# bauerca/maxwell

Measured on NVIDIA B200. Metric: curlcurl_spmv_crs_equiv_gbs, higher is better.
Workload: dtype f64

## Files before the change

### maxwell_b200/csrc/mxg_internal.h

```cpp
#pragma once
#include <cuda_runtime.h>
#include <nccl.h>

#include <cstdarg>
#include <cstdint>
#include <cstdio>
#include <memory>
#include <string>
#include <vector>

#include "mxgpu.h"

namespace mxg {

void setError(const char* fmt, ...);

#define MXG_CUDA(expr)                                                                       \
  do {                                                                                       \
    cudaError_t e_ = (expr);                                                                 \
    if (e_ != cudaSuccess) {                                                                 \
      mxg::setError("%s:%d: %s failed: %s", __FILE__, __LINE__, #expr, cudaGetErrorString(e_)); \
      return MXG_ERR_CUDA;                                                                   \
    }                                                                                        \
  } while (0)
// ... 94 lines not shown
  size_t bytes = 0;
  ~MvStorage();
};

struct mxg_mv {
  mxg_map* map = nullptr;
  bool isComplex = false;
  int ncols = 0;
  int64_t ld = 0;
  std::shared_ptr<MvStorage> storage;
  std::vector<void*> col;
  std::vector<int> baseCol;
};

namespace mxg {
struct HaloPeer {
  int rank = -1;
  int64_t sendCount = 0, sendOffset = 0;
  int64_t recvCount = 0, recvStart = 0;
};
}

struct mxg_crs {
  mxg_ctx* ctx = nullptr;
  mxg_map *rowMap = nullptr, *domMap = nullptr;
  bool isComplex = false;
  int64_t nRows = 0, nLoc = 0, nnz = 0;
  int64_t gLo = 0, gHi = 0;
  int32_t* dRowPat = nullptr;
  int32_t* dPatOff = nullptr;
  void* dPat = nullptr;
  int64_t numPats = 0, dictRows = 0, patEntries = 0;
  int64_t nGen = 0, ellEntries = 0;
  int32_t* dGenRow = nullptr;
  int32_t* dGenLen = nullptr;
  int64_t* dSlicePtr = nullptr;
  int32_t* dCol = nullptr;
  void* dVal = nullptr;
  int64_t intBegin = 0, intEnd = 0, genIntBegin = 0, genIntEnd = 0;
  int64_t ghostRows = 0;
  std::vector<mxg::HaloPeer> peers;
  int32_t* dSendIdx = nullptr;
  int64_t sendTotal = 0;
  mutable void* dSendBuf = nullptr;
  mutable void* dGhost = nullptr;
  mutable int haloCols = 0;
  size_t deviceBytes = 0;
  void* dInvDiag = nullptr;
  int ilv = 1;
  void* dWinTiles = nullptr;
  int winR = 0;
  int winIlv = 1;
  int winMaxVec = 1;
  int64_t winTiles = 0, winValid = 0;
  int64_t winBufElems = 0;
  struct GraphEntry {
    uint64_t key;
    cudaGraphExec_t exec;
    int launches;
  };
  mutable std::vector<GraphEntry> graphs;
  struct P2P {
    bool on = false;
    unsigned long long hostEpoch = 0;
    int capCols = 0;
    void* ghost = nullptr;
    unsigned long long* flags = nullptr;
    unsigned int* done = nullptr;
    void* dArgs = nullptr;
    unsigned long long* trace = nullptr;
    int npeers = 0;
    int peerRank[8];
    void* peerGhost[8];
    unsigned long long* peerFlag[8];
    int64_t remoteStart[8], remoteGTot[8];
    std::vector<void*> opened;
  };
  mutable P2P p2p;
};

namespace mxg {
template <class T>
inline ColTable<T> tableOf(const mxg_mv* mv, int first = 0, int count = -1) {
  ColTable<T> t;
  if (count < 0) count = mv->ncols - first;
  for (int j = 0; j < count; ++j) t.p[j] = static_cast<T*>(mv->col[first + j]);
  return t;
}
int ensureScratch(mxg_ctx* ctx, size_t bytes);
int ensurePinned(mxg_ctx* ctx, size_t bytes);
int allReduceScratch(mxg_ctx* ctx, size_t count);
int mapGlobalCount(mxg_map* map, int64_t* out);
int checkHaloFault(const mxg_ctx* ctx, const char* where);
int crsCreateFromDevice(mxg_map* rowMap, mxg_map* domMap, const int64_t* dRowptr, const int32_t* dCol, const void* dVal, int64_t colBegin,
                        int64_t colFieldSize, const int64_t* colFieldGids, int isComplex, int layout, mxg_crs** out);
inline int gridFor(const mxg_ctx* ctx, int64_t work, int block, int perSM) {
  int64_t need = (work + block - 1) / block;
  int64_t cap = int64_t(ctx->numSMs) * perSM;
  if (need < 1) need = 1;
  return int(need < cap ? need : cap);
}
}
```

### maxwell_b200/csrc/mxg_spmm_win.cuh

```cuda
#pragma once
#include <algorithm>
#include <climits>
#include <cstdint>
#include <vector>

namespace mxg {

constexpr int kWinThreads = 384;

struct alignas(16) WinTile {
  int32_t segLo[3];
  int32_t segLen[3];
  int32_t shift[3];
  int32_t dLo, dHi;
  int32_t valid;
  int32_t total;
  int32_t pad[3];
};
static_assert(sizeof(WinTile) == 64, "WinTile layout");

template <class Delta>
inline std::vector<WinTile> planWinTiles(const int32_t* rowPat, const int32_t* patOff, int64_t numPats, Delta delta, int64_t nRows,
                                         int64_t nLoc, int R, int align, int64_t budgetElems, int64_t* maxTotal, int64_t* validTiles) {
  const int64_t nTiles = (nRows + R - 1) / R;
// ... 42 lines not shown
    if (!a) { a = b; b = 0; }
    const size_t n = ents.size();
    size_t cb[4];
    int ncl;
    if (a && b) { cb[0] = 0; cb[1] = a; cb[2] = b; cb[3] = n; ncl = 3; }
    else if (a) { cb[0] = 0; cb[1] = a; cb[2] = n; ncl = 2; }
    else { cb[0] = 0; cb[1] = n; ncl = 1; }
    int cls[3];
    if (ncl == 3) { cls[0] = 0; cls[1] = 1; cls[2] = 2; W.dLo = int32_t(ents[a].d); W.dHi = int32_t(ents[b - 1].d); }
    else if (ncl == 2) { cls[0] = 1; cls[1] = 2; W.dHi = int32_t(ents[a - 1].d); }
    else cls[0] = 1;
    bool ok = true;
    int64_t lo[3], hi[3];
    for (int c = 0; c < ncl; ++c) {
      lo[c] = INT64_MAX;
      hi[c] = INT64_MIN;
      for (size_t i = cb[c]; i < cb[c + 1]; ++i) { lo[c] = std::min(lo[c], ents[i].lo); hi[c] = std::max(hi[c], ents[i].hi); }
      if (lo[c] < 0 || hi[c] > nLoc) ok = false;
      lo[c] = lo[c] / align * align;
      hi[c] = (hi[c] + align - 1) / align * align;
    }
    int order[3] = {0, 1, 2};
    std::sort(order, order + ncl, [&](int x, int y) { return lo[x] < lo[y]; });
    int64_t total = 0;
    int nseg = 0, segOf[3] = {0, 0, 0};
    int64_t segLo[3] = {0, 0, 0}, segHi[3] = {0, 0, 0}, segOff[3] = {0, 0, 0};
    for (int k = 0; k < ncl && ok; ++k) {
      const int c = order[k];
      if (nseg > 0 && lo[c] <= segHi[nseg - 1]) segHi[nseg - 1] = std::max(segHi[nseg - 1], hi[c]);
      else { segLo[nseg] = lo[c]; segHi[nseg] = hi[c]; ++nseg; }
      segOf[c] = nseg - 1;
    }
    for (int sgi = 0; sgi < nseg && ok; ++sgi) {
      segOff[sgi] = total;
      total += segHi[sgi] - segLo[sgi];
      W.segLo[sgi] = int32_t(segLo[sgi]);
      W.segLen[sgi] = int32_t(segHi[sgi] - segLo[sgi]);
    }
    for (int c = 0; c < ncl && ok; ++c) W.shift[cls[c]] = int32_t(segOff[segOf[c]] - segLo[segOf[c]]);
    if (!ok || total > budgetElems || total >= (int64_t(1) << 30)) {
      W = WinTile{};
      W.dLo = INT_MIN;
      W.dHi = INT_MAX;
      continue;
    }
    W.valid = 1;
    W.total = int32_t(total);
    *maxTotal = std::max<int64_t>(*maxTotal, total);
    ++*validTiles;
  }
  return tiles;
}

#ifdef __CUDACC__
__device__ __forceinline__ uint32_t smemU32(const void* p) { return static_cast<uint32_t>(__cvta_generic_to_shared(p)); }
__device__ __forceinline__ void mbarInit(uint64_t* bar, uint32_t count) {
  asm volatile("mbarrier.init.shared::cta.b64 [%0], %1;" ::"r"(smemU32(bar)), "r"(count) : "memory");
}
__device__ __forceinline__ void mbarFenceInit() {
  asm volatile("fence.mbarrier_init.release.cluster;" ::: "memory");
  asm volatile("fence.proxy.async.shared::cta;" ::: "memory");
}
__device__ __forceinline__ void mbarExpectTx(uint64_t* bar, uint32_t bytes) {
  asm volatile("mbarrier.arrive.expect_tx.shared::cta.b64 _, [%0], %1;" ::"r"(smemU32(bar)), "r"(bytes) : "memory");
}
__device__ __forceinline__ void bulkLoad(void* dstSmem, const void* srcGlobal, uint32_t bytes, uint64_t* bar) {
  asm volatile("cp.async.bulk.shared::cluster.global.mbarrier::complete_tx::bytes [%0], [%1], %2, [%3];" ::"r"(smemU32(dstSmem)),
               "l"(srcGlobal), "r"(bytes), "r"(smemU32(bar))
               : "memory");
}
__device__ __forceinline__ void mbarWait(uint64_t* bar, uint32_t parity) {
  uint32_t done;
  do {
    asm volatile(
        "{\n"
        ".reg .pred p;\n"
        "mbarrier.try_wait.parity.shared::cta.b64 p, [%1], %2;\n"
        "selp.u32 %0, 1, 0, p;\n"
        "}\n"
        : "=r"(done)
        : "r"(smemU32(bar)), "r"(parity)
        : "memory");
  } while (!done);
}
#endif

}
```

### maxwell_b200/csrc/mxg_spmv.cu

```cuda
#include <algorithm>
#include <cstdlib>
#include <cstring>

#include "mxg_internal.h"
#include "mxg_ilv_model.h"
#include "mxg_order.h"
#include "mxg_spmm_win.cuh"
#include "mxg_scan.cuh"

using namespace mxg;

namespace {

constexpr int kBlock = 256;

template <class T>
struct PatEntry;
template <>
struct __align__(16) PatEntry<double> {
  double v;
  int32_t d;
  int32_t pad;
};
template <>
// ... 118 lines not shown
        v[u] = S.val[at];
      }
#pragma unroll
      for (int u = 0; u < kUnroll; ++u)
#pragma unroll
        for (int jj = 0; jj < NV; ++jj)
          xv[u][jj] = loadX<T, GHOST>(X, min(j0 + jj, nvec - 1), c[u]);
#pragma unroll
      for (int u = 0; u < kUnroll; ++u)
        if (k + u < len) {
#pragma unroll
          for (int jj = 0; jj < NV; ++jj) accum(acc[jj], v[u], xv[u][jj]);
        }
    }
    if (row >= 0) {
#pragma unroll
      for (int jj = 0; jj < NV; ++jj)
        if (NV == 1 || j0 + jj < nvec) storeY(Y.p[j0 + jj], row, acc[jj], ep);
    }
  }
}

template <class T, bool GHOST>
__device__ __forceinline__ void sellRowSimple(int64_t i, const SellArgs<T>& S, const XSource<T>& X, const ColTable<T>& Y, int nvec,
                                              const Epilogue<T>& ep) {
  const int64_t row = S.genRow[i];
  if (row < 0) return;
  const int len = S.genLen[i];
  const int64_t base = S.slicePtr[i >> 5] + (i & 31);
  for (int j = 0; j < nvec; ++j) {
    T acc = zeroOf<T>();
    for (int k = 0; k < len; ++k) accum(acc, S.val[base + int64_t(k) * 32], loadX<T, GHOST>(X, j, S.col[base + int64_t(k) * 32]));
    storeY(Y.p[j], row, acc, ep);
  }
}

template <class T, bool GHOST, int NV>
__global__ void __launch_bounds__(kBlock) k_spmm_dict(int64_t rowBegin, int64_t rowEnd, DictArgs<T> D,
                                                      XSource<T> X, ColTable<T> Y, int nvec, Epilogue<T> ep) {
  const int64_t row = rowBegin + blockIdx.x * int64_t(kBlock) + threadIdx.x;
  if (row < rowEnd) dictRow<T, GHOST, NV>(row, D, X, Y, nvec, ep);
}

constexpr int kBlockIlv = 384;
template <class T, bool GHOST, int NV>
__global__ void __launch_bounds__(kBlockIlv) k_spmm_dict_ilv3(int64_t rowBegin, int64_t rowEnd, DictArgs<T> D,
                                                              XSource<T> X, ColTable<T> Y, int nvec, Epilogue<T> ep) {
  const int warp = threadIdx.x >> 5, lane = threadIdx.x & 31;
  const int64_t row = rowBegin + blockIdx.x * int64_t(kBlockIlv) + (warp / 3) * 96 + 3 * lane + (warp % 3);
  if (row < rowEnd) dictRow<T, GHOST, NV>(row, D, X, Y, nvec, ep);
}


template <class T>
__device__ __forceinline__ void winIssue(const WinTile& W, const T* __restrict__ xcol, T* buf, uint64_t* bar) {
  uint32_t bytes = 0;
#pragma unroll
  for (int sgi = 0; sgi < 3; ++sgi) bytes += uint32_t(W.segLen[sgi]) * uint32_t(sizeof(T));
  mbarExpectTx(bar, bytes);
  int off = 0;
#pragma unroll
  for (int sgi = 0; sgi < 3; ++sgi) {
    if (W.segLen[sgi] > 0) bulkLoad(buf + off, xcol + W.segLo[sgi], uint32_t(W.segLen[sgi]) * uint32_t(sizeof(T)), bar);
    off += W.segLen[sgi];
  }
}

constexpr int kWinSlot = 16;

template <class T>
__device__ __forceinline__ PatEntry<T> ldEntry(const PatEntry<T>* p) {
  PatEntry<T> e;
  const int4* s = reinterpret_cast<const int4*>(p);
  int4* d = reinterpret_cast<int4*>(&e);
#pragma unroll
  for (int i = 0; i < int(sizeof(PatEntry<T>) / 16); ++i) d[i] = s[i];
  return e;
}

struct WinShift {
  int32_t dLo, dHi, s0, s1, s2;
};
template <class T>
__device__ __forceinline__ T winRowDot(const PatEntry<T>* __restrict__ ent, int32_t len, int32_t r, const T* __restrict__ xs, const WinShift& w) {
  T acc = zeroOf<T>();
  int32_t q = 0;
  for (; q + 1 < len; q += 2) {
    const PatEntry<T> e0 = ldEntry<T>(ent + q);
    const PatEntry<T> e1 = ldEntry<T>(ent + q + 1);
    const T x0 = xs[r + e0.d + (e0.d < w.dLo ? w.s0 : (e0.d > w.dHi ? w.s2 : w.s1))];
    const T x1 = xs[r + e1.d + (e1.d < w.dLo ? w.s0 : (e1.d > w.dHi ? w.s2 : w.s1))];
    accum(acc, entryVal(e0), x0);
    accum(acc, entryVal(e1), x1);
  }
  if (q < len) {
    const PatEntry<T> e0 = ldEntry<T>(ent + q);
    accum(acc, entryVal(e0), xs[r + e0.d + (e0.d < w.dLo ? w.s0 : (e0.d > w.dHi ? w.s2 : w.s1))]);
  }
  return acc;
}

template <class T, int ILV, int RPT>
__global__ void __launch_bounds__(kWinThreads) k_spmm_win(int64_t rowBegin, int64_t rowEnd, int64_t tile0, DictArgs<T> D,
                                                          const WinTile* __restrict__ tiles, XSource<T> X, ColTable<T> Y, int nvec,
                                                          Epilogue<T> ep) {
  extern __shared__ __align__(128) unsigned char smemRaw[];
  uint64_t* bar = reinterpret_cast<uint64_t*>(smemRaw);
  WinTile* Ws = reinterpret_cast<WinTile*>(smemRaw + 64);
  PatEntry<T>* slots = reinterpret_cast<PatEntry<T>*>(smemRaw + 128);
  constexpr int kWarps = kWinThreads / 32;
  T* buf = reinterpret_cast<T*>(smemRaw + 128 + sizeof(PatEntry<T>) * kWarps * RPT * kWinSlot);
  constexpr int R = kWinThreads * RPT;
  const int64_t tile = tile0 + blockIdx.x;
  if (threadIdx.x == 0) {
    const int4* src = reinterpret_cast<const int4*>(tiles + tile);
    int4* dst = reinterpret_cast<int4*>(Ws);
#pragma unroll
    for (int i = 0; i < 4; ++i) dst[i] = __ldg(src + i);
    mbarInit(bar, 1);
    mbarFenceInit();
    if (Ws->valid) winIssue<T>(*Ws, X.x.p[0], buf, bar);
  }
  const int warp = threadIdx.x >> 5, lane = threadIdx.x & 31;
  const int tOff = ILV == 3 ? (warp / 3) * 96 + 3 * lane + (warp % 3) : int(threadIdx.x);
  int64_t row[RPT];
  int32_t o[RPT], len[RPT];
  bool uni[RPT];
#pragma unroll
  for (int i = 0; i < RPT; ++i) {
    row[i] = tile * R + i * kWinThreads + tOff;
    int32_t p = -1;
    if (row[i] >= rowBegin && row[i] < rowEnd) p = D.rowPat[row[i]];
    o[i] = len[i] = 0;
    if (p >= 0) { o[i] = __ldg(D.patOff + p); len[i] = __ldg(D.patOff + p + 1) - o[i]; }
    const int32_t pmax = __reduce_max_sync(0xffffffffu, p);
    uni[i] = __all_sync(0xffffffffu, p < 0 || p == pmax) && pmax >= 0;
    const int32_t oU = __shfl_sync(0xffffffffu, o[i], __ffs(__ballot_sync(0xffffffffu, p == pmax)) - 1);
    const int32_t lenU = __shfl_sync(0xffffffffu, len[i], __ffs(__ballot_sync(0xffffffffu, p == pmax)) - 1);
    uni[i] = uni[i] && lenU <= kWinSlot;
    if (uni[i] && lane < lenU) slots[(warp * RPT + i) * kWinSlot + lane] = ldEntry<T>(D.pat + oU + lane);
  }
  __syncthreads();
  if (!Ws->valid) {
#pragma unroll
    for (int i = 0; i < RPT; ++i)
      if (row[i] >= rowBegin && row[i] < rowEnd) dictRow<T, false, 1>(row[i], D, X, Y, nvec, ep);
    return;
  }
  const int32_t dLo = Ws->dLo, dHi = Ws->dHi, s0 = Ws->shift[0], s1 = Ws->shift[1], s2 = Ws->shift[2];
  for (int j = 0; j < nvec; ++j) {
    mbarWait(bar, j & 1);
    const T* __restrict__ xs = buf;
#pragma unroll
    for (int i = 0; i < RPT; ++i) {
      if (len[i] == 0) continue;
      const int32_t r = int32_t(row[i]);
      const WinShift ws{dLo, dHi, s0, s1, s2};
      const T acc = uni[i] ? winRowDot<T>(slots + (warp * RPT + i) * kWinSlot, len[i], r, xs, ws)
                           : winRowDot<T>(D.pat + o[i], len[i], r, xs, ws);
      storeY(Y.p[j], row[i], acc, ep);
    }
    if (j + 1 < nvec) {
      __syncthreads();
      if (threadIdx.x == 0) winIssue<T>(*Ws, X.x.p[j + 1], buf, bar);
    }
  }
}

template <class T, bool GHOST, int NV>
__global__ void __launch_bounds__(kBlock) k_spmm_sell(int64_t genBegin, int64_t genEnd, SellArgs<T> S,
                                                      XSource<T> X, ColTable<T> Y, int nvec, Epilogue<T> ep) {
  const int64_t i = genBegin + blockIdx.x * int64_t(kBlock) + threadIdx.x;
  if (i < genEnd) sellRow<T, GHOST, NV>(i, S, X, Y, nvec, ep);
}

struct Segments {
  int64_t begin[4], end[4];
  int blockStart[5];
};
template <class T, bool GHOST, int NV>
__global__ void __launch_bounds__(kBlock) k_spmm_multi(Segments G, DictArgs<T> D, SellArgs<T> S,
                                                       XSource<T> X, ColTable<T> Y, int nvec, Epilogue<T> ep) {
  int seg = 0;
  while (seg < 3 && int(blockIdx.x) >= G.blockStart[seg + 1]) ++seg;
  const int64_t idx = G.begin[seg] + int64_t(int(blockIdx.x) - G.blockStart[seg]) * kBlock + threadIdx.x;
  if (idx >= G.end[seg]) return;
  if (seg < 2) dictRow<T, GHOST, NV>(idx, D, X, Y, nvec, ep);
  else sellRow<T, GHOST, NV>(idx, S, X, Y, nvec, ep);
}

template <class T>
__global__ void __launch_bounds__(kBlock) k_pack(ColTable<T> x, const int32_t* __restrict__ idx, int64_t n, T* __restrict__ buf) {
  const T* __restrict__ c = x.p[blockIdx.y];
  for (int64_t i = blockIdx.x * int64_t(kBlock) + threadIdx.x; i < n; i += int64_t(gridDim.x) * kBlock)
    buf[blockIdx.y * n + i] = c[idx[i]];
}

#define LAUNCH_CHECK(ctx)         \
  do {                            \
    (ctx)->launches++;            \
    MXG_CUDA(cudaGetLastError()); \
  } while (0)

template <class T>
DictArgs<T> dictArgs(const mxg_crs* A) { return {A->dRowPat, A->dPatOff, static_cast<const PatEntry<T>*>(A->dPat)}; }
template <class T>
SellArgs<T> sellArgs(const mxg_crs* A) { return {A->dGenRow, A->dGenLen, A->dSlicePtr, A->dCol, static_cast<const T*>(A->dVal)}; }

template <class T, bool GHOST>
int launchSegments(const mxg_crs* A, const int64_t b[4], const int64_t e[4], const XSource<T>& X, const ColTable<T>& Y, int nvec,
                   const Epilogue<T>& ep, cudaStream_t st) {
  mxg_ctx* ctx = A->ctx;
  Segments G;
  int blocks = 0;
  for (int sgm = 0; sgm < 4; ++sgm) {
    G.begin[sgm] = b[sgm];
    G.end[sgm] = e[sgm] > b[sgm] ? e[sgm] : b[sgm];
    G.blockStart[sgm] = blocks;
    blocks += int((G.end[sgm] - G.begin[sgm] + kBlock - 1) / kBlock);
  }
  G.blockStart[4] = blocks;
  if (blocks == 0) return MXG_OK;
  const DictArgs<T> D = dictArgs<T>(A);
  const SellArgs<T> S = sellArgs<T>(A);
  if (nvec == 1) k_spmm_multi<T, GHOST, 1><<<blocks, kBlock, 0, st>>>(G, D, S, X, Y, nvec, ep);
  else if (nvec == 2) k_spmm_multi<T, GHOST, 2><<<blocks, kBlock, 0, st>>>(G, D, S, X, Y, nvec, ep);
  else k_spmm_multi<T, GHOST, 4><<<blocks, kBlock, 0, st>>>(G, D, S, X, Y, nvec, ep);
  LAUNCH_CHECK(ctx);
  return MXG_OK;
}


template <class T> struct WinCfg;
template <> struct WinCfg<double> { static constexpr int RPT = 2; };
template <> struct WinCfg<zd> { static constexpr int RPT = 1; };
constexpr size_t kWinSmemMax = 200 * 1024;
constexpr size_t kWinBufBudget = 100 * 1024;
template <class T>
constexpr size_t winSmemHeader() { return 128 + sizeof(PatEntry<T>) * (kWinThreads / 32) * WinCfg<T>::RPT * kWinSlot; }

template <class T>
int launchWin(const mxg_crs* A, int64_t rowBegin, int64_t rowEnd, const XSource<T>& X, const ColTable<T>& Y, int nvec,
              const Epilogue<T>& ep, cudaStream_t st) {
  mxg_ctx* ctx = A->ctx;
  constexpr int RPT = WinCfg<T>::RPT;
  const int R = A->winR;
  const int64_t tile0 = rowBegin / R, tiles = (rowEnd + R - 1) / R - tile0;
  const size_t smem = winSmemHeader<T>() + size_t(A->winBufElems) * sizeof(T);
  const DictArgs<T> D = dictArgs<T>(A);
  const WinTile* wt = static_cast<const WinTile*>(A->dWinTiles);
  static bool attrSet[2] = {false, false};
  if (A->winIlv == 3) {
    auto kern = k_spmm_win<T, 3, RPT>;
    if (!attrSet[0]) { MXG_CUDA(cudaFuncSetAttribute(kern, cudaFuncAttributeMaxDynamicSharedMemorySize, int(kWinSmemMax))); attrSet[0] = true; }
    kern<<<unsigned(tiles), kWinThreads, smem, st>>>(rowBegin, rowEnd, tile0, D, wt, X, Y, nvec, ep);
  } else {
    auto kern = k_spmm_win<T, 1, RPT>;
    if (!attrSet[1]) { MXG_CUDA(cudaFuncSetAttribute(kern, cudaFuncAttributeMaxDynamicSharedMemorySize, int(kWinSmemMax))); attrSet[1] = true; }
    kern<<<unsigned(tiles), kWinThreads, smem, st>>>(rowBegin, rowEnd, tile0, D, wt, X, Y, nvec, ep);
  }
  LAUNCH_CHECK(ctx);
  return MXG_OK;
}

template <class T, bool GHOST>
int launchRange(const mxg_crs* A, int64_t rowBegin, int64_t rowEnd, int64_t genBegin, int64_t genEnd, const XSource<T>& X,
                const ColTable<T>& Y, int nvec, const Epilogue<T>& ep, bool marks) {
  mxg_ctx* ctx = A->ctx;
  const cudaStream_t st = ctx->stream;
  if (marks) MXG_CUDA(cudaEventRecord(ctx->prof[1], st));
  if (A->dictRows > 0 && rowEnd > rowBegin && A->winR > 0 && nvec <= A->winMaxVec) {
    const int rc = launchWin<T>(A, rowBegin, rowEnd, X, Y, nvec, ep, st);
    if (rc) return rc;
  } else if (A->dictRows > 0 && rowEnd > rowBegin) {
    const DictArgs<T> D = dictArgs<T>(A);
    if (A->ilv == 3) {
      const int64_t blocks = (rowEnd - rowBegin + kBlockIlv - 1) / kBlockIlv;
      if (nvec == 1) k_spmm_dict_ilv3<T, GHOST, 1><<<blocks, kBlockIlv, 0, st>>>(rowBegin, rowEnd, D, X, Y, nvec, ep);
      else if (nvec == 2) k_spmm_dict_ilv3<T, GHOST, 2><<<blocks, kBlockIlv, 0, st>>>(rowBegin, rowEnd, D, X, Y, nvec, ep);
      else k_spmm_dict_ilv3<T, GHOST, 4><<<blocks, kBlockIlv, 0, st>>>(rowBegin, rowEnd, D, X, Y, nvec, ep);
    } else {
      const int64_t blocks = (rowEnd - rowBegin + kBlock - 1) / kBlock;
      if (nvec == 1) k_spmm_dict<T, GHOST, 1><<<blocks, kBlock, 0, st>>>(rowBegin, rowEnd, D, X, Y, nvec, ep);
      else if (nvec == 2) k_spmm_dict<T, GHOST, 2><<<blocks, kBlock, 0, st>>>(rowBegin, rowEnd, D, X, Y, nvec, ep);
      else k_spmm_dict<T, GHOST, 4><<<blocks, kBlock, 0, st>>>(rowBegin, rowEnd, D, X, Y, nvec, ep);
    }
    LAUNCH_CHECK(ctx);
  }
  if (marks) MXG_CUDA(cudaEventRecord(ctx->prof[2], st));
  if (genEnd > genBegin) {
    const int64_t blocks = (genEnd - genBegin + kBlock - 1) / kBlock;
    const SellArgs<T> S = sellArgs<T>(A);
    if (nvec == 1) k_spmm_sell<T, GHOST, 1><<<blocks, kBlock, 0, st>>>(genBegin, genEnd, S, X, Y, nvec, ep);
    else if (nvec == 2) k_spmm_sell<T, GHOST, 2><<<blocks, kBlock, 0, st>>>(genBegin, genEnd, S, X, Y, nvec, ep);
    else k_spmm_sell<T, GHOST, 4><<<blocks, kBlock, 0, st>>>(genBegin, genEnd, S, X, Y, nvec, ep);
    LAUNCH_CHECK(ctx);
  }
  if (marks) MXG_CUDA(cudaEventRecord(ctx->prof[3], st));
  return MXG_OK;
}

template <class T>
int launchBoundary(const mxg_crs* A, const XSource<T>& X, const ColTable<T>& Y, int nvec, const Epilogue<T>& ep, cudaStream_t st) {
  const int64_t b[4] = {0, A->intEnd, 0, A->genIntEnd};
  const int64_t e[4] = {A->dictRows > 0 ? A->intBegin : 0, A->dictRows > 0 ? A->nRows : A->intEnd, A->genIntBegin, A->nGen};
  return launchSegments<T, true>(A, b, e, X, Y, nvec, ep, st);
}

__host__ __device__ inline uint64_t mix64(uint64_t h, uint64_t v) {
  h ^= v + 0x9E3779B97F4A7C15ull + (h << 6) + (h >> 2);
  h *= 0xBF58476D1CE4E5B9ull;
  return h ^ (h >> 29);
}
// ... 416 lines not shown
    for (int64_t i = 0; i < cnt[q]; ++i) {
      const int64_t g = all[size_t(q) * maxCnt + i];
      if (g >= domLo && g <= domHi) {
        const int32_t l = domLookup[g];
        MXG_REQUIRE(l >= 0, "mxg_crs_create: rank %d asks for GID %lld which lies in rank %d's range but is not in its map",
                    q, (long long)g, ctx->rank);
        sendIdx.push_back(l);
      }
    }
    peer.sendCount = int64_t(sendIdx.size()) - peer.sendOffset;
    const int64_t qLo = ranges[2 * q], qHi = ranges[2 * q + 1];
    if (qLo <= qHi) {
      auto b = std::lower_bound(ghosts.begin(), ghosts.end(), qLo);
      auto e = std::upper_bound(ghosts.begin(), ghosts.end(), qHi);
      peer.recvStart = int64_t(b - ghosts.begin());
      peer.recvCount = int64_t(e - b);
    }
    if (peer.sendCount > 0 || peer.recvCount > 0) A->peers.push_back(peer);
  }
  int64_t covered = 0;
  for (const Peer& p : A->peers) covered += p.recvCount;
  MXG_REQUIRE(covered == int64_t(ghosts.size()), "mxg_crs_create: %lld ghost columns have no owner",
              (long long)(int64_t(ghosts.size()) - covered));
  A->sendTotal = int64_t(sendIdx.size());
  int rcU = uploadVec(sendIdx, &A->dSendIdx, &A->deviceBytes, ctx);
  if (rcU) return rcU;
  return setupP2P(A, int64_t(ghosts.size()));
}

template <class T>
int planKernels(mxg_crs* A, const std::vector<int32_t>& rowPat, const std::vector<int32_t>& patOff, const std::vector<PatEntry<T>>& pat) {
  mxg_ctx* ctx = A->ctx;
  const int64_t nRows = A->nRows, nLoc = A->nLoc;
  int rc = MXG_OK;
  {
    const char* env = std::getenv("MXG_SPMV_ILV");
    const std::string mode = env ? env : "auto";
    A->ilv = 1;
    if (mode == "3") A->ilv = 3;
    else if (mode != "1" && A->dictRows > 0) {
      const PatEntry<T>* pe = pat.data();
      const mxg::IlvCost cost = mxg::ilvCostModel(rowPat.data(), patOff.data(), [pe](int32_t q) { return pe[q].d; }, A->intBegin,
                                                  A->intEnd, int(sizeof(T)), int(sizeof(PatEntry<T>)));
      if (mxg::ilvWins(cost)) A->ilv = 3;
    }
  }

  {
    const char* env = std::getenv("MXG_SPMV_WIN");
    const bool want = !(env && std::strcmp(env, "0") == 0);
    if (want && A->dictRows > 0 && nLoc + A->gLo + A->gHi < (int64_t(1) << 30)) {
      constexpr int R = kWinThreads * WinCfg<T>::RPT;
      constexpr int align = 16 / int(sizeof(T)) > 0 ? 16 / int(sizeof(T)) : 1;
      const PatEntry<T>* pe = pat.data();
      int64_t maxTotal = 0, valid = 0;
      std::vector<WinTile> tiles = planWinTiles(rowPat.data(), patOff.data(), A->numPats, [pe](int32_t q) { return int64_t(pe[q].d); }, nRows,
                                                nLoc, R, align, int64_t(std::min(kWinBufBudget, kWinSmemMax - winSmemHeader<T>()) / sizeof(T)), &maxTotal, &valid);
      if (valid > 0) {
        WinTile* dT = nullptr;
        if ((rc = uploadVec(tiles, &dT, &A->deviceBytes, ctx))) return rc;
        A->dWinTiles = dT;
        A->winR = R;
        A->winTiles = int64_t(tiles.size());
        A->winValid = valid;
        A->winBufElems = maxTotal;
        A->winMaxVec = 1;
        if (const char* mv = std::getenv("MXG_WIN_MAXVEC")) A->winMaxVec = std::atoi(mv);
        int64_t same1 = 0, same3 = 0;
        for (int64_t r = 0; r + 3 < nRows; ++r) {
          if (rowPat[r] < 0) continue;
          same1 += rowPat[r] == rowPat[r + 1];
          same3 += rowPat[r] == rowPat[r + 3];
        }
        A->winIlv = same3 > same1 ? 3 : 1;
        if (const char* iv = std::getenv("MXG_SPMV_ILV")) {
          if (std::strcmp(iv, "1") == 0) A->winIlv = 1;
          if (std::strcmp(iv, "3") == 0) A->winIlv = 3;
        }
      }
    }
  }

  return rc;
}

struct Scratch {
  std::vector<void*> p;
  ~Scratch() { for (void* q : p) if (q) cudaFree(q); }
  template <class U>
  U* get(int64_t n) {
    void* q = nullptr;
    if (cudaMalloc(&q, size_t(n > 0 ? n : 1) * sizeof(U)) != cudaSuccess) { cudaGetLastError(); return nullptr; }
    p.push_back(q);
    return static_cast<U*>(q);
  }
};

constexpr unsigned long long kLbEmpty = 0xFFFFFFFFFFFFFFFFull;

__global__ void k_lb_mark_ghosts(const int32_t* __restrict__ col, int64_t cnt, int64_t c0, int64_t c1, int32_t* __restrict__ flag) {
  for (int64_t q = int64_t(blockIdx.x) * blockDim.x + threadIdx.x; q < cnt; q += int64_t(gridDim.x) * blockDim.x) {
    const int64_t l = col[q];
    if (l < c0 || l >= c1) flag[l] = 1;
  }
}
__global__ void k_lb_compact(const int32_t* __restrict__ flag, const int64_t* __restrict__ off, int64_t n, int32_t* __restrict__ list) {
  for (int64_t i = int64_t(blockIdx.x) * blockDim.x + threadIdx.x; i < n; i += int64_t(gridDim.x) * blockDim.x)
    if (flag[i]) list[off[i]] = int32_t(i);
}
__global__ void k_lb_ext(const int64_t* __restrict__ rp, const int32_t* __restrict__ colG, int64_t nRows, int64_t base, int64_t c0,
                         int64_t c1, int64_t nLoc, int64_t gLo, const int64_t* __restrict__ ghostOff, int32_t* __restrict__ ext,
                         uint8_t* __restrict__ needs, int* __restrict__ err) {
  for (int64_t r = int64_t(blockIdx.x) * blockDim.x + threadIdx.x; r < nRows; r += int64_t(gridDim.x) * blockDim.x) {
    bool ghost = false;
    for (int64_t q = rp[r]; q < rp[r + 1]; ++q) {
      const int64_t l = colG[q];
      int32_t e;
      if (l >= c0 && l < c1) e = int32_t(l - c0);
      else if (ghostOff) {
        const int64_t pos = ghostOff[l];
        e = pos < gLo ? int32_t(pos - gLo) : int32_t(nLoc + (pos - gLo));
        ghost = true;
      } else { *err = 1; e = 0; }
      ext[q - base] = e;
    }
    if (needs) needs[r] = ghost ? 1 : 0;
  }
}

template <class T>
__device__ __forceinline__ uint64_t lbRowHash(const int64_t* rp, const int32_t* ext, const T* valG, int64_t base, int64_t r) {
// ... 773 lines not shown
```

Measured before the change: 15490.

## Make windowed SpMV kernel persistent with double-buffered ring-buffer x windows

Replaces the one-CTA-per-tile windowed SpMV kernel with a persistent kernel that walks a contiguous run of tiles per CTA. The x windows live in a power-of-two ring buffer, so consecutive tiles only fetch the new part of each window. Bulk loads and pattern-entry staging (cp.async) for the next tile overlap with computing the current one. The goal is to cut redundant x reloads and per-tile prologue/launch cost. The price is extra index masking in the inner loop, a more complex host-side plan, and serialisation within each CTA.

```diff
diff --git a/maxwell_b200/csrc/mxg_internal.h b/maxwell_b200/csrc/mxg_internal.h
--- a/maxwell_b200/csrc/mxg_internal.h
+++ b/maxwell_b200/csrc/mxg_internal.h
@@ -170,8 +170,9 @@
   int winR = 0;
   int winIlv = 1;
   int winMaxVec = 1;
+  int winCapLog2 = 0;
+  int64_t winCtas = 0;
   int64_t winTiles = 0, winValid = 0;
-  int64_t winBufElems = 0;
   struct GraphEntry {
     uint64_t key;
     cudaGraphExec_t exec;
diff --git a/maxwell_b200/csrc/mxg_spmm_win.cuh b/maxwell_b200/csrc/mxg_spmm_win.cuh
--- a/maxwell_b200/csrc/mxg_spmm_win.cuh
+++ b/maxwell_b200/csrc/mxg_spmm_win.cuh
@@ -118,6 +118,121 @@
   return tiles;
 }
 
+struct alignas(16) WinRingTile {
+  int32_t dLo, dHi;
+  int32_t flags;
+  int32_t pad;
+  int32_t cls[3][4];
+};
+static_assert(sizeof(WinRingTile) == 64, "WinRingTile layout");
+constexpr int32_t kRingValid = 1, kRingWarm = 2;
+
+#ifdef __CUDACC__
+__host__ __device__
+#endif
+inline int ringCopies(const int32_t cls[4], bool warm, int k, int capLog2, int32_t src[2], int32_t dst[2], int32_t len[2]) {
+  const int32_t C = int32_t(1) << capLog2;
+  const int32_t a = warm ? cls[1] : cls[0], n = cls[2] - a;
+  if (n <= 0) return 0;
+  const int32_t s = a & (C - 1), n0 = n < C - s ? n : C - s;
+  src[0] = a; dst[0] = k * C + s; len[0] = n0;
+  if (n0 == n) return 1;
+  src[1] = a + n0; dst[1] = k * C; len[1] = n - n0;
+  return 2;
+}
+
+struct WinRingPlan {
+  std::vector<WinRingTile> tiles;
+  int capLog2 = 0;
+  int64_t valid = 0, warm = 0;
+  int64_t copied = 0;
+};
+
+template <class Delta>
+inline WinRingPlan planWinRing(const std::vector<WinTile>& wt, const int32_t* rowPat, const int32_t* patOff, int64_t numPats, Delta delta,
+                               int64_t nRows, int R, int align, int maxCapLog2) {
+  const int64_t nTiles = int64_t(wt.size());
+  WinRingPlan P;
+  P.tiles.assign(size_t(nTiles), WinRingTile{});
+  std::vector<int64_t> minRow(size_t(numPats), 0), maxRow(size_t(numPats), 0), stamp(size_t(numPats), -1);
+  std::vector<int32_t> touched;
+  for (int64_t t = 0; t < nTiles; ++t) {
+    WinRingTile& T = P.tiles[size_t(t)];
+    T.dLo = wt[size_t(t)].dLo;
+    T.dHi = wt[size_t(t)].dHi;
+    if (!wt[size_t(t)].valid) continue;
+    const int64_t r0 = t * R, r1 = std::min<int64_t>(nRows, r0 + R);
+    touched.clear();
+    for (int64_t r = r0; r < r1; ++r) {
+      const int32_t p = rowPat[r];
+      if (p < 0) continue;
+      if (stamp[p] != t) { stamp[p] = t; minRow[p] = maxRow[p] = r; touched.push_back(p); }
+      else maxRow[p] = r;
+    }
+    int64_t lo[3] = {INT64_MAX, INT64_MAX, INT64_MAX}, hi[3] = {INT64_MIN, INT64_MIN, INT64_MIN};
+    for (int32_t p : touched)
+      for (int32_t q = patOff[p]; q < patOff[p + 1]; ++q) {
+        const int64_t d = delta(q);
+        const int k = d < T.dLo ? 0 : (d > T.dHi ? 2 : 1);
+        lo[k] = std::min(lo[k], minRow[p] + d);
+        hi[k] = std::max(hi[k], maxRow[p] + d + 1);
+      }
+    for (int k = 0; k < 3; ++k)
+      if (lo[k] < hi[k]) {
+        T.cls[k][0] = int32_t(lo[k] / align * align);
+        T.cls[k][2] = int32_t((hi[k] + align - 1) / align * align);
+      }
+    T.flags = kRingValid;
+  }
+  auto used = [](const WinRingTile& T, int k) { return T.cls[k][0] < T.cls[k][2]; };
+  auto own = [&](const WinRingTile& T) {
+    int64_t w = 0;
+    for (int k = 0; k < 3; ++k) if (used(T, k)) w = std::max<int64_t>(w, T.cls[k][2] - T.cls[k][0]);
+    return w;
+  };
+  auto link = [&](const WinRingTile& A, const WinRingTile& B) {
+    int64_t w = 0;
+    for (int k = 0; k < 3; ++k) {
+      if (!used(A, k) || !used(B, k)) continue;
+      if (B.cls[k][0] < A.cls[k][0] || B.cls[k][2] < A.cls[k][2]) return int64_t(-1);
+      w = std::max<int64_t>(w, int64_t(B.cls[k][2]) - A.cls[k][0]);
+    }
+    return w;
+  };
+  const int64_t capMax = int64_t(1) << maxCapLog2;
+  int64_t need = 1;
+  for (int64_t t = 0; t < nTiles; ++t) {
+    const WinRingTile& T = P.tiles[size_t(t)];
+    if (!(T.flags & kRingValid)) continue;
+    const int64_t o = own(T);
+    if (o <= capMax) need = std::max(need, o);
+    if (t > 0 && (P.tiles[size_t(t - 1)].flags & kRingValid)) {
+      const int64_t l = link(P.tiles[size_t(t - 1)], T);
+      if (l >= 0 && l <= capMax) need = std::max(need, l);
+    }
+  }
+  P.capLog2 = 0;
+  while ((int64_t(1) << P.capLog2) < need) ++P.capLog2;
+  P.capLog2 = std::max(P.capLog2, 4);
+  const int64_t C = int64_t(1) << P.capLog2;
+  bool prevValid = false;
+  for (int64_t t = 0; t < nTiles; ++t) {
+    WinRingTile& T = P.tiles[size_t(t)];
+    if ((T.flags & kRingValid) && own(T) > C) { T.flags = 0; for (auto& c : T.cls) c[0] = c[1] = c[2] = 0; }
+    if (!(T.flags & kRingValid)) { prevValid = false; continue; }
+    const WinRingTile* A = prevValid ? &P.tiles[size_t(t - 1)] : nullptr;
+    const int64_t l = A ? link(*A, T) : -1;
+    const bool warm = l >= 0 && l <= C;
+    if (warm) T.flags |= kRingWarm;
+    for (int k = 0; k < 3; ++k) T.cls[k][1] = warm && used(*A, k) ? A->cls[k][2] : T.cls[k][0];
+    for (int k = 0; k < 3; ++k) P.copied += T.cls[k][2] - T.cls[k][warm ? 1 : 0];
+    ++P.valid;
+    P.warm += warm;
+    prevValid = true;
+  }
+  return P;
+}
+
 #ifdef __CUDACC__
 __device__ __forceinline__ uint32_t smemU32(const void* p) { return static_cast<uint32_t>(__cvta_generic_to_shared(p)); }
 __device__ __forceinline__ void mbarInit(uint64_t* bar, uint32_t count) {
@@ -149,6 +264,11 @@
         : "memory");
   } while (!done);
 }
+__device__ __forceinline__ void fenceProxyAsync() { asm volatile("fence.proxy.async.shared::cta;" ::: "memory"); }
+__device__ __forceinline__ void cpAsync16(void* dstSmem, const void* srcGlobal) {
+  asm volatile("cp.async.cg.shared.global [%0], [%1], 16;" ::"r"(smemU32(dstSmem)), "l"(srcGlobal) : "memory");
+}
+__device__ __forceinline__ void cpAsyncWaitAll() { asm volatile("cp.async.wait_all;" ::: "memory"); }
 #endif
 
 }
diff --git a/maxwell_b200/csrc/mxg_spmv.cu b/maxwell_b200/csrc/mxg_spmv.cu
--- a/maxwell_b200/csrc/mxg_spmv.cu
+++ b/maxwell_b200/csrc/mxg_spmv.cu
@@ -194,20 +194,6 @@
 }
 
 
-template <class T>
-__device__ __forceinline__ void winIssue(const WinTile& W, const T* __restrict__ xcol, T* buf, uint64_t* bar) {
-  uint32_t bytes = 0;
-#pragma unroll
-  for (int sgi = 0; sgi < 3; ++sgi) bytes += uint32_t(W.segLen[sgi]) * uint32_t(sizeof(T));
-  mbarExpectTx(bar, bytes);
-  int off = 0;
-#pragma unroll
-  for (int sgi = 0; sgi < 3; ++sgi) {
-    if (W.segLen[sgi] > 0) bulkLoad(buf + off, xcol + W.segLo[sgi], uint32_t(W.segLen[sgi]) * uint32_t(sizeof(T)), bar);
-    off += W.segLen[sgi];
-  }
-}
-
 constexpr int kWinSlot = 16;
 
 template <class T>
@@ -221,90 +207,166 @@
 }
 
 struct WinShift {
-  int32_t dLo, dHi, s0, s1, s2;
+  int32_t dLo, dHi, cap, cap2, mask;
 };
+__device__ __forceinline__ int32_t ringIdx(int32_t r, int32_t d, const WinShift& w) {
+  return (d < w.dLo ? 0 : (d > w.dHi ? w.cap2 : w.cap)) + ((r + d) & w.mask);
+}
 template <class T>
 __device__ __forceinline__ T winRowDot(const PatEntry<T>* __restrict__ ent, int32_t len, int32_t r, const T* __restrict__ xs, const WinShift& w) {
   T acc = zeroOf<T>();
   int32_t q = 0;
-  for (; q + 1 < len; q += 2) {
+  if (sizeof(T) == 8) {
+#pragma unroll 1
+    for (; q + 1 < len; q += 2) {
+      const PatEntry<T> e0 = ldEntry<T>(ent + q);
+      const PatEntry<T> e1 = ldEntry<T>(ent + q + 1);
+      const T x0 = xs[ringIdx(r, e0.d, w)];
+      const T x1 = xs[ringIdx(r, e1.d, w)];
+      accum(acc, entryVal(e0), x0);
+      accum(acc, entryVal(e1), x1);
+    }
+  }
+#pragma unroll 1
+  for (; q < len; ++q) {
     const PatEntry<T> e0 = ldEntry<T>(ent + q);
-    const PatEntry<T> e1 = ldEntry<T>(ent + q + 1);
-    const T x0 = xs[r + e0.d + (e0.d < w.dLo ? w.s0 : (e0.d > w.dHi ? w.s2 : w.s1))];
-    const T x1 = xs[r + e1.d + (e1.d < w.dLo ? w.s0 : (e1.d > w.dHi ? w.s2 : w.s1))];
-    accum(acc, entryVal(e0), x0);
-    accum(acc, entryVal(e1), x1);
-  }
-  if (q < len) {
-    const PatEntry<T> e0 = ldEntry<T>(ent + q);
-    accum(acc, entryVal(e0), xs[r + e0.d + (e0.d < w.dLo ? w.s0 : (e0.d > w.dHi ? w.s2 : w.s1))]);
+    accum(acc, entryVal(e0), xs[ringIdx(r, e0.d, w)]);
   }
   return acc;
 }
 
+template <int RPT>
+struct WinRows {
+  int32_t o[RPT], len[RPT];
+  bool uni[RPT];
+};
+template <class T, int RPT>
+__device__ __forceinline__ void winPats(int64_t t, int64_t tEnd, int tOff, int64_t rowBegin, int64_t rowEnd, const DictArgs<T>& D,
+                                        int32_t (&p)[RPT]) {
+#pragma unroll
+  for (int i = 0; i < RPT; ++i) {
+    const int64_t row = t * (kWinThreads * RPT) + i * kWinThreads + tOff;
+    p[i] = t < tEnd && row >= rowBegin && row < rowEnd ? __ldg(D.rowPat + row) : -1;
+  }
+}
+template <class T, int RPT>
+__device__ __forceinline__ void winPrep(const DictArgs<T>& D, const int32_t (&p)[RPT], PatEntry<T>* slot, int lane, WinRows<RPT>& w) {
+#pragma unroll
+  for (int i = 0; i < RPT; ++i) {
+    w.o[i] = w.len[i] = 0;
+    if (p[i] >= 0) { w.o[i] = __ldg(D.patOff + p[i]); w.len[i] = __ldg(D.patOff + p[i] + 1) - w.o[i]; }
+    const int32_t pmax = __reduce_max_sync(0xffffffffu, p[i]);
+    const int src = __ffs(__ballot_sync(0xffffffffu, p[i] == pmax)) - 1;
+    const int32_t oU = __shfl_sync(0xffffffffu, w.o[i], src);
+    const int32_t lenU = __shfl_sync(0xffffffffu, w.len[i], src);
+    w.uni[i] = __all_sync(0xffffffffu, p[i] < 0 || p[i] == pmax) && pmax >= 0 && lenU <= kWinSlot;
+    if (w.uni[i] && lane < lenU) {
+      const char* s = reinterpret_cast<const char*>(D.pat + oU + lane);
+      char* d = reinterpret_cast<char*>(slot + i * kWinSlot + lane);
+#pragma unroll
+      for (int b = 0; b < int(sizeof(PatEntry<T>)); b += 16) cpAsync16(d + b, s + b);
+    }
+  }
+}
+template <class T>
+__device__ __forceinline__ void winRingIssue(const int4& cls, bool warm, int capLog2, const T* xcol, T* ring, uint64_t* bar, int lane) {
+  int32_t src[2], dst[2], len[2];
+  int n = 0;
+  if (lane < 3) {
+    const int32_t c[4] = {cls.x, cls.y, cls.z, cls.w};
+    n = ringCopies(c, warm, lane, capLog2, src, dst, len);
+  }
+  uint32_t bytes = 0;
+#pragma unroll
+  for (int i = 0; i < 2; ++i)
+    if (i < n) bytes += uint32_t(len[i]) * uint32_t(sizeof(T));
+  bytes = __reduce_add_sync(0xffffffffu, bytes);
+  if (lane == 0) mbarExpectTx(bar, bytes);
+  __syncwarp();
+#pragma unroll
+  for (int i = 0; i < 2; ++i)
+    if (i < n) bulkLoad(ring + dst[i], xcol + src[i], uint32_t(len[i]) * uint32_t(sizeof(T)), bar);
+}
+
+__device__ __forceinline__ void winRecord(const WinRingTile* __restrict__ tiles, int64_t t, int64_t tEnd, WinRingTile* rec, int warp, int lane) {
+  if (warp == 0 && lane < 4 && t < tEnd) cpAsync16(reinterpret_cast<int4*>(rec) + lane, reinterpret_cast<const int4*>(tiles + t) + lane);
+}
+constexpr int kWinHeader = 320;
+
 template <class T, int ILV, int RPT>
-__global__ void __launch_bounds__(kWinThreads) k_spmm_win(int64_t rowBegin, int64_t rowEnd, int64_t tile0, DictArgs<T> D,
-                                                          const WinTile* __restrict__ tiles, XSource<T> X, ColTable<T> Y, int nvec,
-                                                          Epilogue<T> ep) {
+__global__ void __launch_bounds__(kWinThreads, 2) k_spmm_win(int64_t rowBegin, int64_t rowEnd, DictArgs<T> D,
+                                                             const WinRingTile* __restrict__ tiles, int capLog2, XSource<T> X,
+                                                             ColTable<T> Y, int nvec, Epilogue<T> ep) {
   extern __shared__ __align__(128) unsigned char smemRaw[];
+  constexpr int kWarps = kWinThreads / 32, R = kWinThreads * RPT, kStage = kWarps * RPT * kWinSlot;
   uint64_t* bar = reinterpret_cast<uint64_t*>(smemRaw);
-  WinTile* Ws = reinterpret_cast<WinTile*>(smemRaw + 64);
-  PatEntry<T>* slots = reinterpret_cast<PatEntry<T>*>(smemRaw + 128);
-  constexpr int kWarps = kWinThreads / 32;
-  T* buf = reinterpret_cast<T*>(smemRaw + 128 + sizeof(PatEntry<T>) * kWarps * RPT * kWinSlot);
-  constexpr int R = kWinThreads * RPT;
-  const int64_t tile = tile0 + blockIdx.x;
-  if (threadIdx.x == 0) {
-    const int4* src = reinterpret_cast<const int4*>(tiles + tile);
-    int4* dst = reinterpret_cast<int4*>(Ws);
-#pragma unroll
-    for (int i = 0; i < 4; ++i) dst[i] = __ldg(src + i);
-    mbarInit(bar, 1);
-    mbarFenceInit();
-    if (Ws->valid) winIssue<T>(*Ws, X.x.p[0], buf, bar);
-  }
+  WinRingTile* recs = reinterpret_cast<WinRingTile*>(smemRaw + 128);
+  PatEntry<T>* slots = reinterpret_cast<PatEntry<T>*>(smemRaw + kWinHeader);
+  T* ring = reinterpret_cast<T*>(smemRaw + kWinHeader + sizeof(PatEntry<T>) * 2 * kStage);
   const int warp = threadIdx.x >> 5, lane = threadIdx.x & 31;
   const int tOff = ILV == 3 ? (warp / 3) * 96 + 3 * lane + (warp % 3) : int(threadIdx.x);
-  int64_t row[RPT];
-  int32_t o[RPT], len[RPT];
-  bool uni[RPT];
-#pragma unroll
-  for (int i = 0; i < RPT; ++i) {
-    row[i] = tile * R + i * kWinThreads + tOff;
-    int32_t p = -1;
-    if (row[i] >= rowBegin && row[i] < rowEnd) p = D.rowPat[row[i]];
-    o[i] = len[i] = 0;
-    if (p >= 0) { o[i] = __ldg(D.patOff + p); len[i] = __ldg(D.patOff + p + 1) - o[i]; }
-    const int32_t pmax = __reduce_max_sync(0xffffffffu, p);
-    uni[i] = __all_sync(0xffffffffu, p < 0 || p == pmax) && pmax >= 0;
-    const int32_t oU = __shfl_sync(0xffffffffu, o[i], __ffs(__ballot_sync(0xffffffffu, p == pmax)) - 1);
-    const int32_t lenU = __shfl_sync(0xffffffffu, len[i], __ffs(__ballot_sync(0xffffffffu, p == pmax)) - 1);
-    uni[i] = uni[i] && lenU <= kWinSlot;
-    if (uni[i] && lane < lenU) slots[(warp * RPT + i) * kWinSlot + lane] = ldEntry<T>(D.pat + oU + lane);
-  }
-  __syncthreads();
-  if (!Ws->valid) {
-#pragma unroll
-    for (int i = 0; i < RPT; ++i)
-      if (row[i] >= rowBegin && row[i] < rowEnd) dictRow<T, false, 1>(row[i], D, X, Y, nvec, ep);
-    return;
-  }
-  const int32_t dLo = Ws->dLo, dHi = Ws->dHi, s0 = Ws->shift[0], s1 = Ws->shift[1], s2 = Ws->shift[2];
+  const int64_t tile0 = rowBegin / R, nT = (rowEnd + R - 1) / R - tile0;
+  const int64_t cBeg = tile0 + nT * blockIdx.x / gridDim.x, cEnd = tile0 + nT * (blockIdx.x + 1) / gridDim.x;
+  if (cBeg >= cEnd) return;
+  if (threadIdx.x == 0) {
+    mbarInit(bar, 1);
+    mbarInit(bar + 1, 1);
+    mbarFenceInit();
+  }
+  WinShift w{0, 0, int32_t(1) << capLog2, int32_t(2) << capLog2, (int32_t(1) << capLog2) - 1};
+  uint32_t phase = 0;
   for (int j = 0; j < nvec; ++j) {
-    mbarWait(bar, j & 1);
-    const T* __restrict__ xs = buf;
-#pragma unroll
-    for (int i = 0; i < RPT; ++i) {
-      if (len[i] == 0) continue;
-      const int32_t r = int32_t(row[i]);
-      const WinShift ws{dLo, dHi, s0, s1, s2};
-      const T acc = uni[i] ? winRowDot<T>(slots + (warp * RPT + i) * kWinSlot, len[i], r, xs, ws)
-                           : winRowDot<T>(D.pat + o[i], len[i], r, xs, ws);
-      storeY(Y.p[j], row[i], acc, ep);
-    }
-    if (j + 1 < nvec) {
+    const T* __restrict__ xcol = X.x.p[j];
+    int64_t t = cBeg;
+    winRecord(tiles, t, cEnd, recs, warp, lane);
+    winRecord(tiles, t + 1, cEnd, recs + 1, warp, lane);
+    int32_t p[RPT];
+    winPats<T, RPT>(t, cEnd, tOff, rowBegin, rowEnd, D, p);
+    WinRows<RPT> cur;
+    winPrep<T, RPT>(D, p, slots + warp * RPT * kWinSlot, lane, cur);
+    winPats<T, RPT>(t + 1, cEnd, tOff, rowBegin, rowEnd, D, p);
+    cpAsyncWaitAll();
+    __syncthreads();
+    if (warp == 0 && (recs[0].flags & kRingValid))
+      winRingIssue<T>(reinterpret_cast<const int4*>(recs)[1 + lane % 3], false, capLog2, xcol, ring, bar, lane);
+    for (int s = 0, rc = 0; t < cEnd; ++t, s ^= 1, rc = rc == 2 ? 0 : rc + 1) {
+      const int rn = rc == 2 ? 0 : rc + 1, rnn = rn == 2 ? 0 : rn + 1;
+      const int32_t flagsN = t + 1 < cEnd ? recs[rn].flags : 0;
+      const bool validN = flagsN & kRingValid, warmN = validN && (flagsN & kRingWarm);
+      if (warp == 0 && warmN)
+        winRingIssue<T>(reinterpret_cast<const int4*>(recs + rn)[1 + lane % 3], true, capLog2, xcol, ring, bar + (s ^ 1), lane);
+      WinRows<RPT> nxt;
+      winPrep<T, RPT>(D, p, slots + ((s ^ 1) * kWarps + warp) * RPT * kWinSlot, lane, nxt);
+      winRecord(tiles, t + 2, cEnd, recs + rnn, warp, lane);
+      winPats<T, RPT>(t + 2, cEnd, tOff, rowBegin, rowEnd, D, p);
+      const int32_t flags = recs[rc].flags;
+      if (flags & kRingValid) {
+        w.dLo = recs[rc].dLo;
+        w.dHi = recs[rc].dHi;
+        mbarWait(bar + s, (phase >> s) & 1u);
+        phase ^= 1u << s;
+        const PatEntry<T>* slot = slots + (s * kWarps + warp) * RPT * kWinSlot;
+#pragma unroll
+        for (int i = 0; i < RPT; ++i) {
+          if (cur.len[i] == 0) continue;
+          const int64_t row = t * R + i * kWinThreads + tOff;
+          const T acc = cur.uni[i] ? winRowDot<T>(slot + i * kWinSlot, cur.len[i], int32_t(row), ring, w)
+                                   : winRowDot<T>(D.pat + cur.o[i], cur.len[i], int32_t(row), ring, w);
+          storeY(Y.p[j], row, acc, ep);
+        }
+      } else if (j == 0) {
+#pragma unroll
+        for (int i = 0; i < RPT; ++i) {
+          const int64_t row = t * R + i * kWinThreads + tOff;
+          if (row >= rowBegin && row < rowEnd) dictRow<T, false, 1>(row, D, X, Y, nvec, ep);
+        }
+      }
+      fenceProxyAsync();
+      cpAsyncWaitAll();
       __syncthreads();
-      if (threadIdx.x == 0) winIssue<T>(*Ws, X.x.p[j + 1], buf, bar);
+      if (warp == 0 && validN && !warmN)
+        winRingIssue<T>(reinterpret_cast<const int4*>(recs + rn)[1 + lane % 3], false, capLog2, xcol, ring, bar + (s ^ 1), lane);
+      cur = nxt;
     }
   }
 }
@@ -376,31 +438,44 @@
 template <class T> struct WinCfg;
 template <> struct WinCfg<double> { static constexpr int RPT = 2; };
 template <> struct WinCfg<zd> { static constexpr int RPT = 1; };
-constexpr size_t kWinSmemMax = 200 * 1024;
-constexpr size_t kWinBufBudget = 100 * 1024;
-template <class T>
-constexpr size_t winSmemHeader() { return 128 + sizeof(PatEntry<T>) * (kWinThreads / 32) * WinCfg<T>::RPT * kWinSlot; }
+constexpr size_t kWinRingBytes = 96 * 1024;
+template <class T>
+constexpr int winMaxCapLog2() {
+  int l = 0;
+  while (3 * (size_t(2) << l) * sizeof(T) <= kWinRingBytes) ++l;
+  return l;
+}
+template <class T>
+constexpr size_t winSmemHeader() { return kWinHeader + 2 * sizeof(PatEntry<T>) * (kWinThreads / 32) * WinCfg<T>::RPT * kWinSlot; }
+template <class T>
+size_t winSmem(int capLog2) { return winSmemHeader<T>() + 3 * (size_t(1) << capLog2) * sizeof(T); }
+
+template <class T>
+using WinKernel = void (*)(int64_t, int64_t, DictArgs<T>, const WinRingTile*, int, XSource<T>, ColTable<T>, int, Epilogue<T>);
+template <class T>
+WinKernel<T> winKernel(int ilv) {
+  constexpr int RPT = WinCfg<T>::RPT;
+  const WinKernel<T> k = ilv == 3 ? k_spmm_win<T, 3, RPT> : k_spmm_win<T, 1, RPT>;
+  static bool attrSet[2] = {false, false};
+  if (!attrSet[ilv == 3]) {
+    const int smemMax = int(winSmem<T>(winMaxCapLog2<T>()));
+    if (cudaFuncSetAttribute(k, cudaFuncAttributeMaxDynamicSharedMemorySize, smemMax) != cudaSuccess) return nullptr;
+    attrSet[ilv == 3] = true;
+  }
+  return k;
+}
 
 template <class T>
 int launchWin(const mxg_crs* A, int64_t rowBegin, int64_t rowEnd, const XSource<T>& X, const ColTable<T>& Y, int nvec,
               const Epilogue<T>& ep, cudaStream_t st) {
   mxg_ctx* ctx = A->ctx;
-  constexpr int RPT = WinCfg<T>::RPT;
   const int R = A->winR;
-  const int64_t tile0 = rowBegin / R, tiles = (rowEnd + R - 1) / R - tile0;
-  const size_t smem = winSmemHeader<T>() + size_t(A->winBufElems) * sizeof(T);
-  const DictArgs<T> D = dictArgs<T>(A);
-  const WinTile* wt = static_cast<const WinTile*>(A->dWinTiles);
-  static bool attrSet[2] = {false, false};
-  if (A->winIlv == 3) {
-    auto kern = k_spmm_win<T, 3, RPT>;
-    if (!attrSet[0]) { MXG_CUDA(cudaFuncSetAttribute(kern, cudaFuncAttributeMaxDynamicSharedMemorySize, int(kWinSmemMax))); attrSet[0] = true; }
-    kern<<<unsigned(tiles), kWinThreads, smem, st>>>(rowBegin, rowEnd, tile0, D, wt, X, Y, nvec, ep);
-  } else {
-    auto kern = k_spmm_win<T, 1, RPT>;
-    if (!attrSet[1]) { MXG_CUDA(cudaFuncSetAttribute(kern, cudaFuncAttributeMaxDynamicSharedMemorySize, int(kWinSmemMax))); attrSet[1] = true; }
-    kern<<<unsigned(tiles), kWinThreads, smem, st>>>(rowBegin, rowEnd, tile0, D, wt, X, Y, nvec, ep);
-  }
+  const int64_t tiles = (rowEnd + R - 1) / R - rowBegin / R;
+  const WinKernel<T> kern = winKernel<T>(A->winIlv);
+  MXG_REQUIRE(kern != nullptr, "mxg_crs_apply: cannot give the windowed SpMM kernel %zu bytes of shared memory", winSmem<T>(winMaxCapLog2<T>()));
+  const unsigned grid = unsigned(std::min<int64_t>(tiles, A->winCtas));
+  kern<<<grid, kWinThreads, winSmem<T>(A->winCapLog2), st>>>(rowBegin, rowEnd, dictArgs<T>(A), static_cast<const WinRingTile*>(A->dWinTiles),
+                                                             A->winCapLog2, X, Y, nvec, ep);
   LAUNCH_CHECK(ctx);
   return MXG_OK;
 }
@@ -923,20 +998,15 @@
     if (want && A->dictRows > 0 && nLoc + A->gLo + A->gHi < (int64_t(1) << 30)) {
       constexpr int R = kWinThreads * WinCfg<T>::RPT;
       constexpr int align = 16 / int(sizeof(T)) > 0 ? 16 / int(sizeof(T)) : 1;
+      constexpr int maxCapLog2 = winMaxCapLog2<T>();
       const PatEntry<T>* pe = pat.data();
+      auto delta = [pe](int32_t q) { return int64_t(pe[q].d); };
       int64_t maxTotal = 0, valid = 0;
-      std::vector<WinTile> tiles = planWinTiles(rowPat.data(), patOff.data(), A->numPats, [pe](int32_t q) { return int64_t(pe[q].d); }, nRows,
-                                                nLoc, R, align, int64_t(std::min(kWinBufBudget, kWinSmemMax - winSmemHeader<T>()) / sizeof(T)), &maxTotal, &valid);
-      if (valid > 0) {
-        WinTile* dT = nullptr;
-        if ((rc = uploadVec(tiles, &dT, &A->deviceBytes, ctx))) return rc;
-        A->dWinTiles = dT;
-        A->winR = R;
-        A->winTiles = int64_t(tiles.size());
-        A->winValid = valid;
-        A->winBufElems = maxTotal;
-        A->winMaxVec = 1;
-        if (const char* mv = std::getenv("MXG_WIN_MAXVEC")) A->winMaxVec = std::atoi(mv);
+      const std::vector<WinTile> tiles = planWinTiles(rowPat.data(), patOff.data(), A->numPats, delta, nRows, nLoc, R, align,
+                                                      int64_t(3) << maxCapLog2, &maxTotal, &valid);
+      const WinRingPlan ring = valid > 0 ? planWinRing(tiles, rowPat.data(), patOff.data(), A->numPats, delta, nRows, R, align, maxCapLog2)
+                                         : WinRingPlan{};
+      if (ring.valid > 0) {
         int64_t same1 = 0, same3 = 0;
         for (int64_t r = 0; r + 3 < nRows; ++r) {
           if (rowPat[r] < 0) continue;
@@ -948,6 +1018,23 @@
           if (std::strcmp(iv, "1") == 0) A->winIlv = 1;
           if (std::strcmp(iv, "3") == 0) A->winIlv = 3;
         }
+        const WinKernel<T> kern = winKernel<T>(A->winIlv);
+        MXG_REQUIRE(kern != nullptr, "mxg_crs_create: cannot give the windowed SpMM kernel %zu bytes of shared memory", winSmem<T>(maxCapLog2));
+        int dev = 0, sms = 0, perSm = 0;
+        MXG_CUDA(cudaGetDevice(&dev));
+        MXG_CUDA(cudaDeviceGetAttribute(&sms, cudaDevAttrMultiProcessorCount, dev));
+        MXG_CUDA(cudaOccupancyMaxActiveBlocksPerMultiprocessor(&perSm, kern, kWinThreads, winSmem<T>(ring.capLog2)));
+        A->winCtas = int64_t(sms) * std::max(perSm, 1);
+        if (const char* nc = std::getenv("MXG_WIN_CTAS")) A->winCtas = std::max(1, std::atoi(nc));
+        WinRingTile* dT = nullptr;
+        if ((rc = uploadVec(ring.tiles, &dT, &A->deviceBytes, ctx))) return rc;
+        A->dWinTiles = dT;
+        A->winR = R;
+        A->winTiles = int64_t(ring.tiles.size());
+        A->winValid = ring.valid;
+        A->winCapLog2 = ring.capLog2;
+        A->winMaxVec = 1;
+        if (const char* mv = std::getenv("MXG_WIN_MAXVEC")) A->winMaxVec = std::atoi(mv);
       }
     }
   }
```

New measurement: 9277 (median of 6 runs). 40.1% lower.
